# Cornell-RelaxML/QuIP

Measured on NVIDIA H100. Metric: tokens/sec 2-bit Llama-2-7B (per-layer eval path, seq 2048), higher is better.
Workload: dtype f16

## Files before the change

quip_b200/csrc/qgemm_tc.cu:

```cuda
#include <type_traits>

#include "tc_common.cuh"

namespace quip {

constexpr int TC_SMEM_MAX = 227 * 1024;

template <int BITS, int BN, bool DENSE, int RB = 1>
struct TcCfg {
  static constexpr int BM = TC_BM * RB;
  static constexpr int A_BYTES = DENSE ? TC_BM * TC_BK * 2 : (BM / SB_ROWS) * sb_words(BITS) * 4;
  static constexpr int B_BYTES = BN * TC_BK * 2;
  static constexpr int STAGE_BYTES = A_BYTES + B_BYTES;
  static constexpr int EPI_HALVES = BN * 72 > 64 * (BN + 8) ? BN * 72 : 64 * (BN + 8);
  static constexpr int EPI_BYTES = 2 * EPI_HALVES * 2;
  static constexpr int STAGES_FIT = (TC_SMEM_MAX - EPI_BYTES - 1024 - 256) / STAGE_BYTES;
  static constexpr int STAGES = STAGES_FIT < 16 ? STAGES_FIT : 16;
  static constexpr size_t SMEM = (size_t)STAGES * STAGE_BYTES + 1024  + 256  + EPI_BYTES;
  static_assert(STAGE_BYTES % 1024 == 0 && 2 * STAGES * 8 <= 256, "stage layout");
  static_assert(RB == 1 || (!DENSE && BN == 128), "256-row tiles: packed GEMM at BN = 128 only");
};

template <int BITS, int BN, bool DENSE, int RB = 1>
__global__ void __launch_bounds__(RB == 1 ? TC_THREADS : TC_THREADS_TALL, 1)
qgemm_tc_kernel(const __grid_constant__ CUtensorMap tmap_x, const __grid_constant__ CUtensorMap tmap_a,
                const float* __restrict__ scales, const float* __restrict__ zeros, const __half* __restrict__ bias,
                const float* __restrict__ xsum, __half* __restrict__ z, int M, int K, int N, int symmetric, int nblk,
                int shared_factor) {
  using C = TcCfg<BITS, BN, DENSE, RB>;
  extern __shared__ unsigned char smem_raw[];
  const uint32_t smem_base = (smem_u32(smem_raw) + 1023u) & ~1023u;
  unsigned char* smem_gen = smem_raw + (smem_base - smem_u32(smem_raw));
  uint64_t* bars = reinterpret_cast<uint64_t*>(smem_gen + (size_t)C::STAGES * C::STAGE_BYTES);
  uint64_t* full = bars;
  uint64_t* empty = bars + C::STAGES;
  __half* epi = reinterpret_cast<__half*>(smem_gen + (size_t)C::STAGES * C::STAGE_BYTES + 256);

  const int warp = threadIdx.x >> 5, lane = threadIdx.x & 31;
  const int tiles_n = DENSE ? (N + BN - 1) / BN : (N + C::BM - 1) / C::BM;
  const int tiles_m = DENSE ? (M + TC_BM - 1) / TC_BM : (M + BN - 1) / BN;
  const int per_blk = tiles_n * tiles_m;
  const int num_tiles = per_blk * nblk;
  const int KB = (K + TC_BK - 1) / TC_BK;
  const int64_t ldz = (int64_t)N * nblk;
  constexpr int TMA_WARP = TC_CONSUMER_WARPS;

  if (warp == TMA_WARP && lane == 0) {
    asm volatile("prefetch.tensormap [%0];" ::"l"(&tmap_x) : "memory");
    asm volatile("prefetch.tensormap [%0];" ::"l"(&tmap_a) : "memory");
    for (int s = 0; s < C::STAGES; ++s) {
      mbar_init(&full[s], 1);
      mbar_init(&empty[s], TC_CONSUMER_WARPS);
    }
    asm volatile("fence.mbarrier_init.release.cluster;" ::: "memory");
  }
  __syncthreads();

  if (RB == 1 ? warp == TMA_WARP : warp >= TMA_WARP) {
    if constexpr (RB == 2) asm volatile("setmaxnreg.dec.sync.aligned.u32 %0;" ::"n"(TC_TALL_PRODUCER_REGS));
    if (lane == 0 && (RB == 1 || warp == TMA_WARP)) {
      int s = 0;
      uint32_t ph = 0;
      for (int tile = blockIdx.x; tile < num_tiles; tile += gridDim.x) {
        const int blk = tile / per_blk, rr = tile % per_blk;
        const int m0 = (rr / tiles_n) * (DENSE ? TC_BM : BN), n0 = (rr % tiles_n) * (DENSE ? BN : C::BM);
        for (int kb = 0; kb < KB; ++kb) {
          mbar_wait(&empty[s], ph ^ 1u);
          unsigned char* stage = smem_gen + (size_t)s * C::STAGE_BYTES;
          if (DENSE) {
            mbar_arrive_expect_tx(&full[s], C::STAGE_BYTES);
            tma_load_2d(stage, &tmap_x, &full[s], blk * K + kb * TC_BK, m0);
            tma_load_3d(stage + C::A_BYTES, &tmap_a, &full[s], kb * TC_BK, n0, shared_factor ? 0 : blk);
          } else {
            const bool words = (kb & 1) == 0;
            mbar_arrive_expect_tx(&full[s], C::B_BYTES + (words ? C::A_BYTES : 0));
            if (words) tma_load_2d(stage, &tmap_a, &full[s], (kb >> 1) * sb_words(BITS), n0 / SB_ROWS);
            tma_load_2d(stage + C::A_BYTES, &tmap_x, &full[s], kb * TC_BK, m0);
          }
          if (++s == C::STAGES) { s = 0; ph ^= 1u; }
        }
      }
    }
  } else {
    if constexpr (RB == 2) asm volatile("setmaxnreg.inc.sync.aligned.u32 %0;" ::"n"(TC_TALL_CONSUMER_REGS));
    const int wg = warp >> 2, wtid = threadIdx.x & 127;
    const int frow = (warp & 3) * 16 + (lane >> 2);
    const int fcol = (lane & 3) * 2;
    __half* eb = epi + wg * C::EPI_HALVES;
    float acc[RB][BN / 2];
#pragma unroll
    for (int j = 0; j < BN / 2; ++j) acc[0][j] = 0.f;
    int s = 0;
    uint32_t ph = 0;
    auto advance = [&]() { if (++s == C::STAGES) { s = 0; ph ^= 1u; } };
    auto release = [&](int st) {
      __syncwarp();
      if (lane == 0) mbar_arrive(&empty[st]);
    };
    for (int tile = blockIdx.x; tile < num_tiles; tile += gridDim.x) {
      const int blk = tile / per_blk, rr = tile % per_blk;
      int prev = 0;
      const int n_base = (rr % tiles_n) * C::BM + wg * 64 * RB, m0 = (rr / tiles_n) * BN;
      float Pn[RB][2], Rn[RB][2], bn[RB][2];
      if constexpr (!DENSE) {
#pragma unroll
        for (int hf = 0; hf < RB; ++hf)
#pragma unroll
          for (int h = 0; h < 2; ++h) {
            const int n = n_base + 64 * hf + frow + 8 * h;
            Pn[hf][h] = 1.f; Rn[hf][h] = 0.f; bn[hf][h] = 0.f;
            if (n < N) {
              const float sc = scales[n];
              Pn[hf][h] = sc * (float)(1 << BITS);
              if (!symmetric) Rn[hf][h] = sc * (0.5f * (float)((1 << BITS) - 1)) - zeros[n];
              if (bias) bn[hf][h] = __half2float(bias[n]);
            }
          }
        if (!symmetric && wtid < BN / 32 && m0 + 32 * wtid < M)
          asm volatile("prefetch.global.L1 [%0];" ::"l"(xsum + m0 + 32 * wtid));
      }
      if constexpr (DENSE) {
        for (int kb = 0; kb < KB; ++kb) {
          mbar_wait(&full[s], ph);
          const uint32_t a_addr = smem_base + (uint32_t)(s * C::STAGE_BYTES);
          const uint64_t adesc = make_sw128_desc(a_addr + (uint32_t)(wg * 64 * 128));
          const uint64_t bdesc = make_sw128_desc(a_addr + C::A_BYTES);
          wgmma_fence();
#pragma unroll
          for (int k = 0; k < TC_BK / 16; ++k)
            wgmma_f16_ss<BN>(acc[0], adesc + (uint64_t)(2 * k), bdesc + (uint64_t)(2 * k), (kb | k) ? 1 : 0);
          wgmma_commit();
          wgmma_wait<1>();
          if (kb > 0) release(prev);
          prev = s;
          advance();
        }
      } else if constexpr (RB == 1) {
        const int g = lane >> 2, t = lane & 3;
        const uint32_t row_off = (uint32_t)(warp * sb_words(BITS) * 4);
        uint32_t w[row_words(BITS)];
        uint32_t fa[2][16];
        auto issue = [&](const uint32_t (&f)[16], int first) {
          const uint64_t bdesc = make_sw128_desc(smem_base + (uint32_t)(s * C::STAGE_BYTES) + C::A_BYTES);
          wgmma_fence();
#pragma unroll
          for (int k = 0; k < TC_BK / 16; ++k)
            wgmma_f16_rs<BN>(acc[0], &f[4 * k], bdesc + (uint64_t)(2 * k), (first && k == 0) ? 0 : 1);
          wgmma_commit();
        };
        auto load_words = [&]() {
          mbar_wait(&full[s], ph);
          tc_load_row_words<BITS>(smem_base + (uint32_t)(s * C::STAGE_BYTES) + row_off, g, w);
        };
        load_words();
        frag_natural<BITS, 0, 0>(w, t, &fa[0][0]);
        frag_natural<BITS, 0, 1>(w, t, &fa[0][4]);
        frag_natural<BITS, 1, 0>(w, t, &fa[0][8]);
        frag_natural<BITS, 1, 1>(w, t, &fa[0][12]);
        const int KSB = KB >> 1;
        for (int ksb = 0; ksb < KSB; ++ksb) {
          const int se = s;
          issue(fa[0], ksb == 0);
          wgmma_wait<1>();
          if (ksb > 0) release(prev);
          advance();
          mbar_wait(&full[s], ph);
          frag_natural<BITS, 2, 0>(w, t, &fa[1][0]);
          frag_natural<BITS, 2, 1>(w, t, &fa[1][4]);
          frag_natural<BITS, 3, 0>(w, t, &fa[1][8]);
          frag_natural<BITS, 3, 1>(w, t, &fa[1][12]);
          issue(fa[1], 0);
          wgmma_wait<1>();
          release(se);
          prev = s;
          advance();
          if (ksb + 1 < KSB) {
            load_words();
            frag_natural<BITS, 0, 0>(w, t, &fa[0][0]);
            frag_natural<BITS, 0, 1>(w, t, &fa[0][4]);
            frag_natural<BITS, 1, 0>(w, t, &fa[0][8]);
            frag_natural<BITS, 1, 1>(w, t, &fa[0][12]);
          }
        }
      } else {
        const int g = lane >> 2, t = lane & 3;
        const uint32_t row_off0 = (uint32_t)((wg * 8 + (warp & 3)) * sb_words(BITS) * 4);
        const uint32_t row_off1 = row_off0 + (uint32_t)(4 * sb_words(BITS) * 4);
        uint32_t w[row_words(BITS)];
        uint32_t fa[2][16];
        auto issue = [&](const uint32_t (&f)[16], float (&d)[BN / 2], int first) {
          const uint64_t bdesc = make_sw128_desc(smem_base + (uint32_t)(s * C::STAGE_BYTES) + C::A_BYTES);
          wgmma_fence();
#pragma unroll
          for (int k = 0; k < TC_BK / 16; ++k)
            wgmma_f16_rs<BN>(d, &f[4 * k], bdesc + (uint64_t)(2 * k), (first && k == 0) ? 0 : 1);
          wgmma_commit();
        };
        auto build = [&](auto odd, int se, uint32_t off, uint32_t (&f)[16]) {
          tc_load_row_words<BITS>(smem_base + (uint32_t)(se * C::STAGE_BYTES) + off, g, w);
          constexpr int c0 = decltype(odd)::value ? 2 : 0;
          frag_natural<BITS, c0, 0>(w, t, &f[0]);
          frag_natural<BITS, c0, 1>(w, t, &f[4]);
          frag_natural<BITS, c0 + 1, 0>(w, t, &f[8]);
          frag_natural<BITS, c0 + 1, 1>(w, t, &f[12]);
        };
        using Even = std::false_type;
        using Odd = std::true_type;
        mbar_wait(&full[s], ph);
        build(Even{}, s, row_off0, fa[0]);
        const int KSB = KB >> 1;
        for (int ksb = 0; ksb < KSB; ++ksb) {
          const int se = s;
          issue(fa[0], acc[0], ksb == 0);
          wgmma_wait<1>();
          if (ksb > 0) release(prev);
          build(Even{}, se, row_off1, fa[1]);
          issue(fa[1], acc[1], ksb == 0);
          wgmma_wait<1>();
          build(Odd{}, se, row_off0, fa[0]);
          advance();
          mbar_wait(&full[s], ph);
          issue(fa[0], acc[0], 0);
          wgmma_wait<1>();
          build(Odd{}, se, row_off1, fa[1]);
          release(se);
          issue(fa[1], acc[1], 0);
          wgmma_wait<1>();
          prev = s;
          advance();
          if (ksb + 1 < KSB) {
            mbar_wait(&full[s], ph);
            build(Even{}, s, row_off0, fa[0]);
          }
        }
      }
      wgmma_wait<0>();
      wgmma_fence_regs(acc[0]);
      if constexpr (RB == 2) wgmma_fence_regs(acc[RB - 1]);
      release(prev);

      if constexpr (DENSE) {
        constexpr int EP = BN + 8;
#pragma unroll
        for (int j = 0; j < BN / 2; j += 2) {
          const int r = frow + ((j & 2) ? 8 : 0), c = 8 * (j >> 2) + fcol;
          *reinterpret_cast<__half2*>(&eb[r * EP + c]) = __floats2half2_rn(acc[0][j], acc[0][j + 1]);
        }
        asm volatile("bar.sync %0, 128;" ::"r"(1 + wg) : "memory");
        const int m_base = (rr / tiles_n) * TC_BM + wg * 64, i0 = (rr % tiles_n) * BN;
        for (int idx = wtid; idx < 64 * (BN / 8); idx += 128) {
          const int r = idx / (BN / 8), v = idx % (BN / 8);
          const int m = m_base + r, i = i0 + 8 * v;
          if (m < M && i < N)
            *reinterpret_cast<uint4*>(z + (int64_t)m * ldz + (int64_t)blk * N + i) =
                *reinterpret_cast<const uint4*>(&eb[r * EP + 8 * v]);
        }
      } else {
        constexpr int EP = 72;
#pragma unroll
        for (int hf = 0; hf < RB; ++hf) {
#pragma unroll
          for (int j = 0; j < BN / 2; ++j) {
            const int h = (j >> 1) & 1, c = 8 * (j >> 2) + fcol + (j & 1), m = m0 + c;
            float v = Pn[hf][h] * acc[hf][j] + bn[hf][h];
            if (!symmetric) v += Rn[hf][h] * (m < M ? __ldg(&xsum[m]) : 0.f);
            eb[c * EP + frow + 8 * h] = __float2half_rn(v);
          }
          asm volatile("bar.sync %0, 128;" ::"r"(1 + wg) : "memory");
          for (int idx = wtid; idx < BN * 8; idx += 128) {
            const int c = idx >> 3, v = idx & 7;
            const int m = m0 + c, n = n_base + 64 * hf + 8 * v;
            if (m < M && n < N)
              *reinterpret_cast<uint4*>(z + (int64_t)m * ldz + n) = *reinterpret_cast<const uint4*>(&eb[c * EP + 8 * v]);
          }
          if (hf + 1 < RB) asm volatile("bar.sync %0, 128;" ::"r"(1 + wg) : "memory");
        }
      }
      asm volatile("bar.sync %0, 128;" ::"r"(1 + wg) : "memory");
    }
  }
}

typedef CUresult (*PFN_encodeTiled)(CUtensorMap*, CUtensorMapDataType, cuuint32_t, void*, const cuuint64_t*,
                                    const cuuint64_t*, const cuuint32_t*, const cuuint32_t*, CUtensorMapInterleave,
                                    CUtensorMapSwizzle, CUtensorMapL2promotion, CUtensorMapFloatOOBfill);

static PFN_encodeTiled get_encode() {
  static PFN_encodeTiled fn = nullptr;
  if (!fn) {
    void* p = nullptr;
    cudaDriverEntryPointQueryResult qres;
    if (cudaGetDriverEntryPoint("cuTensorMapEncodeTiled", &p, cudaEnableDefault, &qres) == cudaSuccess &&
        qres == cudaDriverEntryPointSuccess)
      fn = (PFN_encodeTiled)p;
  }
  return fn;
}

static int g_num_sms = 0;

int num_sms() {
  if (!g_num_sms) {
    int dev = 0;
    if (cudaGetDevice(&dev) != cudaSuccess ||
        cudaDeviceGetAttribute(&g_num_sms, cudaDevAttrMultiProcessorCount, dev) != cudaSuccess)
      g_num_sms = 132;
  }
  return g_num_sms;
}

int make_act_map(CUtensorMap* tmap, const void* x, int64_t rows, int64_t cols, int box_rows) {
  PFN_encodeTiled enc = get_encode();
  if (!enc) {
    set_error("cuTensorMapEncodeTiled is not available from the driver");
    return QUIP_ERR_CUDA;
  }
  cuuint64_t dims[2] = {(cuuint64_t)cols, (cuuint64_t)rows};
  cuuint64_t strides[1] = {(cuuint64_t)cols * sizeof(__half)};
  cuuint32_t box[2] = {(cuuint32_t)TC_BK, (cuuint32_t)box_rows};
  cuuint32_t estr[2] = {1, 1};
  CUresult r = enc(tmap, CU_TENSOR_MAP_DATA_TYPE_FLOAT16, 2, (void*)x, dims, strides, box, estr,
                   CU_TENSOR_MAP_INTERLEAVE_NONE, CU_TENSOR_MAP_SWIZZLE_128B, CU_TENSOR_MAP_L2_PROMOTION_L2_256B,
                   CU_TENSOR_MAP_FLOAT_OOB_FILL_NONE);
  if (r != CUDA_SUCCESS) {
    set_error("cuTensorMapEncodeTiled failed with CUresult %d (ptr=%p rows=%lld cols=%lld)", (int)r, x,
              (long long)rows, (long long)cols);
    return QUIP_ERR_CUDA;
  }
  return QUIP_OK;
}

static int make_words_map(CUtensorMap* tmap, const QuipLinearDesc* d, int rows) {
  PFN_encodeTiled enc = get_encode();
  if (!enc) {
    set_error("cuTensorMapEncodeTiled is not available from the driver");
    return QUIP_ERR_CUDA;
  }
  const int sbw = sb_words(d->bits);
  cuuint64_t dims[2] = {(cuuint64_t)(d->K / SB_K) * sbw, (cuuint64_t)(d->N / SB_ROWS)};
  cuuint64_t strides[1] = {dims[0] * sizeof(uint32_t)};
  cuuint32_t box[2] = {(cuuint32_t)sbw, (cuuint32_t)(rows / SB_ROWS)};
  cuuint32_t estr[2] = {1, 1};
  CUresult r = enc(tmap, CU_TENSOR_MAP_DATA_TYPE_UINT32, 2, (void*)d->qweight, dims, strides, box, estr,
                   CU_TENSOR_MAP_INTERLEAVE_NONE, CU_TENSOR_MAP_SWIZZLE_NONE, CU_TENSOR_MAP_L2_PROMOTION_L2_256B,
                   CU_TENSOR_MAP_FLOAT_OOB_FILL_NONE);
  if (r != CUDA_SUCCESS) {
    set_error("cuTensorMapEncodeTiled (packed words) failed with CUresult %d (N=%d K=%d bits=%d)", (int)r, d->N, d->K,
              d->bits);
    return QUIP_ERR_CUDA;
  }
  return QUIP_OK;
}

template <int BITS, int BN, int RB = 1>
static int launch_tc(const QuipLinearDesc* d, const __half* x, const float* xsum, const __half* bias, __half* z,
                     int M, cudaStream_t s) {
  using C = TcCfg<BITS, BN, false, RB>;
  CUtensorMap tmx, tmq;
  if (int e = make_act_map(&tmx, x, M, d->K, BN)) return e;
  if (int e = make_words_map(&tmq, d, C::BM)) return e;
  auto kern = qgemm_tc_kernel<BITS, BN, false, RB>;
  QUIP_CUDA(cudaFuncSetAttribute(kern, cudaFuncAttributeMaxDynamicSharedMemorySize, (int)C::SMEM));
  int tiles = ceil_div(d->N, C::BM) * ceil_div(M, BN);
  int grid = tiles < num_sms() ? tiles : num_sms();
  kern<<<grid, RB == 1 ? TC_THREADS : TC_THREADS_TALL, C::SMEM, s>>>(tmx, tmq, d->scales, d->zeros, bias, xsum, z, M, d->K, d->N,
                                         (d->flags & QUIP_FLAG_SYMMETRIC) ? 1 : 0, 1, 0);
  QUIP_LAUNCHED("qgemm_tc_kernel");
  return QUIP_OK;
}

template <int BN>
static int launch_tc_dense(const QuipPass* ps, const __half* in, __half* out, int M, int n, cudaStream_t s) {
  using C = TcCfg<2, BN, true>;
  PFN_encodeTiled enc = get_encode();
  CUtensorMap tmx, tma;
  if (int e = make_act_map(&tmx, in, M, n, TC_BM)) return e;
  const int p = ps->p;
  cuuint64_t dims[3] = {(cuuint64_t)p, (cuuint64_t)p, (cuuint64_t)(ps->shared ? 1 : ps->nblk)};
  cuuint64_t strides[2] = {(cuuint64_t)p * sizeof(__half), (cuuint64_t)p * p * sizeof(__half)};
  cuuint32_t box[3] = {(cuuint32_t)TC_BK, (cuuint32_t)BN, 1};
  cuuint32_t estr[3] = {1, 1, 1};
  CUresult r = enc(&tma, CU_TENSOR_MAP_DATA_TYPE_FLOAT16, 3, (void*)ps->factors, dims, strides, box, estr,
                   CU_TENSOR_MAP_INTERLEAVE_NONE, CU_TENSOR_MAP_SWIZZLE_128B, CU_TENSOR_MAP_L2_PROMOTION_L2_256B,
                   CU_TENSOR_MAP_FLOAT_OOB_FILL_NONE);
  if (r != CUDA_SUCCESS) {
    set_error("cuTensorMapEncodeTiled (factors) failed with CUresult %d (p=%d nblk=%d)", (int)r, p, ps->nblk);
    return QUIP_ERR_CUDA;
  }
  auto kern = qgemm_tc_kernel<2, BN, true>;
  QUIP_CUDA(cudaFuncSetAttribute(kern, cudaFuncAttributeMaxDynamicSharedMemorySize, (int)C::SMEM));
  int tiles = ceil_div(p, BN) * ceil_div(M, TC_BM) * ps->nblk;
  int grid = tiles < num_sms() ? tiles : num_sms();
  kern<<<grid, TC_THREADS, C::SMEM, s>>>(tmx, tma, nullptr, nullptr, nullptr, nullptr, out, M, p, p, 1,
                                         ps->nblk, ps->shared ? 1 : 0);
  QUIP_LAUNCHED("qgemm_tc_kernel<dense>");
  return QUIP_OK;
}

int pass_big_tc(const QuipPass* ps, const __half* in, __half* out, int64_t M, int n, cudaStream_t s) {
  QUIP_CHECK_ARG(!ps->strided && ps->p % 8 == 0 && n % 8 == 0, "tensor-core pass needs contiguous blocks, p %% 8 == 0");
  QUIP_CHECK_ARG((((uintptr_t)in | (uintptr_t)out | (uintptr_t)ps->factors) & 15) == 0, "tensor-core pass: unaligned pointer");
  return launch_tc_dense<128>(ps, in, out, (int)M, n, s);
}

int g_tc_rows = 0;

int qgemm_tc(const QuipLinearDesc* d, const __half* x, const float* xsum, const __half* bias, __half* z, int M,
             cudaStream_t s) {
  QUIP_CHECK_ARG((((uintptr_t)x | (uintptr_t)d->qweight) & 15) == 0,
                 "tensor-core path needs 16-byte aligned activations and packed words");
  const bool wide = M > 64;
  if (d->bits == 2 && wide) {
    const bool tall = g_tc_rows == 0 ? ceil_div(d->N, 2 * TC_BM) * ceil_div(M, 128) >= num_sms() : g_tc_rows == 256;
    return tall ? launch_tc<2, 128, 2>(d, x, xsum, bias, z, M, s) : launch_tc<2, 128>(d, x, xsum, bias, z, M, s);
  }
#define QUIP_TC(B)                                                            \
  if (d->bits == B)                                                           \
    return wide ? launch_tc<B, 128>(d, x, xsum, bias, z, M, s) : launch_tc<B, 64>(d, x, xsum, bias, z, M, s);
  QUIP_TC(2) QUIP_TC(3) QUIP_TC(4)
#undef QUIP_TC
  set_error("tensor-core kernel: unsupported bits=%d", d->bits);
  return QUIP_ERR_UNSUPPORTED;
}

}
```

quip_b200/csrc/tc_common.cuh:

```cuda
#pragma once
#include <cuda.h>

#include "common.cuh"

namespace quip {

constexpr int TC_BM = 128;
constexpr int TC_BK = 64;
constexpr int TC_CONSUMER_WARPS = 8;
constexpr int TC_THREADS = 32 * TC_CONSUMER_WARPS + 32;
constexpr int TC_THREADS_TALL = 32 * TC_CONSUMER_WARPS + 128;
constexpr int TC_TALL_PRODUCER_REGS = 40;
constexpr int TC_TALL_CONSUMER_REGS = 232;
constexpr uint32_t TC_WATCHDOG = 1u << 28;

__device__ __forceinline__ void mbar_init(uint64_t* bar, uint32_t count) {
  asm volatile("mbarrier.init.shared::cta.b64 [%0], %1;" ::"r"(smem_u32(bar)), "r"(count));
}
__device__ __forceinline__ void mbar_wait(uint64_t* bar, uint32_t parity) {
  uint32_t addr = smem_u32(bar), done = 0, spins = 0;
  while (true) {
    asm volatile(
        "{\n\t.reg .pred p;\n\t"
        "mbarrier.try_wait.parity.shared::cta.b64 p, [%1], %2;\n\t"
        "selp.u32 %0, 1, 0, p;\n\t}"
        : "=r"(done)
        : "r"(addr), "r"(parity)
        : "memory");
    if (done) break;
    if (++spins > TC_WATCHDOG) __trap();
  }
}
__device__ __forceinline__ void mbar_arrive(uint64_t* bar) {
  asm volatile("mbarrier.arrive.shared::cta.b64 _, [%0];" ::"r"(smem_u32(bar)) : "memory");
}
__device__ __forceinline__ void mbar_arrive_expect_tx(uint64_t* bar, uint32_t bytes) {
  asm volatile("mbarrier.arrive.expect_tx.shared::cta.b64 _, [%0], %1;" ::"r"(smem_u32(bar)), "r"(bytes) : "memory");
}
__device__ __forceinline__ void tma_load_2d(void* smem_dst, const CUtensorMap* map, uint64_t* bar, int c0, int c1) {
  asm volatile(
      "cp.async.bulk.tensor.2d.shared::cluster.global.mbarrier::complete_tx::bytes [%0], [%1, {%3, %4}], [%2];"
      ::"r"(smem_u32(smem_dst)), "l"(map), "r"(smem_u32(bar)), "r"(c0), "r"(c1)
      : "memory");
}
__device__ __forceinline__ void tma_load_3d(void* smem_dst, const CUtensorMap* map, uint64_t* bar, int c0, int c1, int c2) {
  asm volatile(
      "cp.async.bulk.tensor.3d.shared::cluster.global.mbarrier::complete_tx::bytes [%0], [%1, {%3, %4, %5}], [%2];"
      ::"r"(smem_u32(smem_dst)), "l"(map), "r"(smem_u32(bar)), "r"(c0), "r"(c1), "r"(c2)
      : "memory");
}

__device__ __forceinline__ uint64_t make_sw128_desc(uint32_t smem_addr) {
  uint64_t d = 0;
  d |= (uint64_t)((smem_addr & 0x3FFFFu) >> 4);
  d |= (uint64_t)1 << 16;
  d |= (uint64_t)(1024 >> 4) << 32;
  d |= (uint64_t)1 << 62;
  return d;
}

template <int N>
__device__ __forceinline__ void wgmma_f16_ss(float (&d)[N / 2], uint64_t adesc, uint64_t bdesc, int scale_d);
template <>
__device__ __forceinline__ void wgmma_f16_ss<64>(float (&d)[32], uint64_t adesc, uint64_t bdesc, int scale_d) {
  asm volatile(
      "{\n\t.reg .pred p;\n\t"
      "setp.ne.b32 p, %34, 0;\n\t"
      "wgmma.mma_async.sync.aligned.m64n64k16.f32.f16.f16 "
      "{%0,%1,%2,%3,%4,%5,%6,%7,%8,%9,%10,%11,%12,%13,%14,%15,%16,%17,%18,%19,%20,%21,%22,%23,%24,%25,%26,%27,%28,%29,%30,%31}, "
      "%32, %33, p, 1, 1, 0, 0;\n\t}"
      : "+f"(d[0]), "+f"(d[1]), "+f"(d[2]), "+f"(d[3]), "+f"(d[4]), "+f"(d[5]), "+f"(d[6]), "+f"(d[7]), "+f"(d[8]), "+f"(d[9]), "+f"(d[10]), "+f"(d[11]), "+f"(d[12]), "+f"(d[13]), "+f"(d[14]), "+f"(d[15]), "+f"(d[16]), "+f"(d[17]), "+f"(d[18]), "+f"(d[19]), "+f"(d[20]), "+f"(d[21]), "+f"(d[22]), "+f"(d[23]), "+f"(d[24]), "+f"(d[25]), "+f"(d[26]), "+f"(d[27]), "+f"(d[28]), "+f"(d[29]), "+f"(d[30]), "+f"(d[31])
      : "l"(adesc), "l"(bdesc), "r"(scale_d));
}

template <>
__device__ __forceinline__ void wgmma_f16_ss<128>(float (&d)[64], uint64_t adesc, uint64_t bdesc, int scale_d) {
  asm volatile(
      "{\n\t.reg .pred p;\n\t"
      "setp.ne.b32 p, %66, 0;\n\t"
      "wgmma.mma_async.sync.aligned.m64n128k16.f32.f16.f16 "
      "{%0,%1,%2,%3,%4,%5,%6,%7,%8,%9,%10,%11,%12,%13,%14,%15,%16,%17,%18,%19,%20,%21,%22,%23,%24,%25,%26,%27,%28,%29,%30,%31,%32,%33,%34,%35,%36,%37,%38,%39,%40,%41,%42,%43,%44,%45,%46,%47,%48,%49,%50,%51,%52,%53,%54,%55,%56,%57,%58,%59,%60,%61,%62,%63}, "
      "%64, %65, p, 1, 1, 0, 0;\n\t}"
      : "+f"(d[0]), "+f"(d[1]), "+f"(d[2]), "+f"(d[3]), "+f"(d[4]), "+f"(d[5]), "+f"(d[6]), "+f"(d[7]), "+f"(d[8]), "+f"(d[9]), "+f"(d[10]), "+f"(d[11]), "+f"(d[12]), "+f"(d[13]), "+f"(d[14]), "+f"(d[15]), "+f"(d[16]), "+f"(d[17]), "+f"(d[18]), "+f"(d[19]), "+f"(d[20]), "+f"(d[21]), "+f"(d[22]), "+f"(d[23]), "+f"(d[24]), "+f"(d[25]), "+f"(d[26]), "+f"(d[27]), "+f"(d[28]), "+f"(d[29]), "+f"(d[30]), "+f"(d[31]), "+f"(d[32]), "+f"(d[33]), "+f"(d[34]), "+f"(d[35]), "+f"(d[36]), "+f"(d[37]), "+f"(d[38]), "+f"(d[39]), "+f"(d[40]), "+f"(d[41]), "+f"(d[42]), "+f"(d[43]), "+f"(d[44]), "+f"(d[45]), "+f"(d[46]), "+f"(d[47]), "+f"(d[48]), "+f"(d[49]), "+f"(d[50]), "+f"(d[51]), "+f"(d[52]), "+f"(d[53]), "+f"(d[54]), "+f"(d[55]), "+f"(d[56]), "+f"(d[57]), "+f"(d[58]), "+f"(d[59]), "+f"(d[60]), "+f"(d[61]), "+f"(d[62]), "+f"(d[63])
      : "l"(adesc), "l"(bdesc), "r"(scale_d));
}
__device__ __forceinline__ void wgmma_fence() { asm volatile("wgmma.fence.sync.aligned;" ::: "memory"); }
__device__ __forceinline__ void wgmma_commit() { asm volatile("wgmma.commit_group.sync.aligned;" ::: "memory"); }
template <int PENDING>
__device__ __forceinline__ void wgmma_wait() { asm volatile("wgmma.wait_group.sync.aligned %0;" ::"n"(PENDING) : "memory"); }
template <int R>
__device__ __forceinline__ void wgmma_fence_regs(float (&d)[R]) {
#pragma unroll
  for (int i = 0; i < R; ++i) asm volatile("" : "+f"(d[i])::"memory");
}

template <int N>
__device__ __forceinline__ void wgmma_f16_rs(float (&d)[N / 2], const uint32_t* a, uint64_t bdesc, int scale_d);
template <>
__device__ __forceinline__ void wgmma_f16_rs<64>(float (&d)[32], const uint32_t* a, uint64_t bdesc, int scale_d) {
  asm volatile(
      "{\n\t.reg .pred p;\n\t"
      "setp.ne.b32 p, %37, 0;\n\t"
      "wgmma.mma_async.sync.aligned.m64n64k16.f32.f16.f16 "
      "{%0,%1,%2,%3,%4,%5,%6,%7,%8,%9,%10,%11,%12,%13,%14,%15,%16,%17,%18,%19,%20,%21,%22,%23,%24,%25,%26,%27,%28,%29,%30,%31}, "
      "{%32,%33,%34,%35}, %36, p, 1, 1, 0;\n\t}"
      : "+f"(d[0]), "+f"(d[1]), "+f"(d[2]), "+f"(d[3]), "+f"(d[4]), "+f"(d[5]), "+f"(d[6]), "+f"(d[7]), "+f"(d[8]), "+f"(d[9]), "+f"(d[10]), "+f"(d[11]), "+f"(d[12]), "+f"(d[13]), "+f"(d[14]), "+f"(d[15]), "+f"(d[16]), "+f"(d[17]), "+f"(d[18]), "+f"(d[19]), "+f"(d[20]), "+f"(d[21]), "+f"(d[22]), "+f"(d[23]), "+f"(d[24]), "+f"(d[25]), "+f"(d[26]), "+f"(d[27]), "+f"(d[28]), "+f"(d[29]), "+f"(d[30]), "+f"(d[31])
      : "r"(a[0]), "r"(a[1]), "r"(a[2]), "r"(a[3]), "l"(bdesc), "r"(scale_d));
}
template <>
__device__ __forceinline__ void wgmma_f16_rs<128>(float (&d)[64], const uint32_t* a, uint64_t bdesc, int scale_d) {
  asm volatile(
      "{\n\t.reg .pred p;\n\t"
      "setp.ne.b32 p, %69, 0;\n\t"
      "wgmma.mma_async.sync.aligned.m64n128k16.f32.f16.f16 "
      "{%0,%1,%2,%3,%4,%5,%6,%7,%8,%9,%10,%11,%12,%13,%14,%15,%16,%17,%18,%19,%20,%21,%22,%23,%24,%25,%26,%27,%28,%29,%30,%31,%32,%33,%34,%35,%36,%37,%38,%39,%40,%41,%42,%43,%44,%45,%46,%47,%48,%49,%50,%51,%52,%53,%54,%55,%56,%57,%58,%59,%60,%61,%62,%63}, "
      "{%64,%65,%66,%67}, %68, p, 1, 1, 0;\n\t}"
      : "+f"(d[0]), "+f"(d[1]), "+f"(d[2]), "+f"(d[3]), "+f"(d[4]), "+f"(d[5]), "+f"(d[6]), "+f"(d[7]), "+f"(d[8]), "+f"(d[9]), "+f"(d[10]), "+f"(d[11]), "+f"(d[12]), "+f"(d[13]), "+f"(d[14]), "+f"(d[15]), "+f"(d[16]), "+f"(d[17]), "+f"(d[18]), "+f"(d[19]), "+f"(d[20]), "+f"(d[21]), "+f"(d[22]), "+f"(d[23]), "+f"(d[24]), "+f"(d[25]), "+f"(d[26]), "+f"(d[27]), "+f"(d[28]), "+f"(d[29]), "+f"(d[30]), "+f"(d[31]), "+f"(d[32]), "+f"(d[33]), "+f"(d[34]), "+f"(d[35]), "+f"(d[36]), "+f"(d[37]), "+f"(d[38]), "+f"(d[39]), "+f"(d[40]), "+f"(d[41]), "+f"(d[42]), "+f"(d[43]), "+f"(d[44]), "+f"(d[45]), "+f"(d[46]), "+f"(d[47]), "+f"(d[48]), "+f"(d[49]), "+f"(d[50]), "+f"(d[51]), "+f"(d[52]), "+f"(d[53]), "+f"(d[54]), "+f"(d[55]), "+f"(d[56]), "+f"(d[57]), "+f"(d[58]), "+f"(d[59]), "+f"(d[60]), "+f"(d[61]), "+f"(d[62]), "+f"(d[63])
      : "r"(a[0]), "r"(a[1]), "r"(a[2]), "r"(a[3]), "l"(bdesc), "r"(scale_d));
}

template <int BITS>
__device__ __forceinline__ void tc_load_row_words(uint32_t rb, int g, uint32_t (&w)[row_words(BITS)]) {
  auto ld4 = [](uint32_t addr, uint32_t* d) {
    asm volatile("ld.shared.v4.b32 {%0,%1,%2,%3}, [%4];" : "=r"(d[0]), "=r"(d[1]), "=r"(d[2]), "=r"(d[3]) : "r"(addr));
  };
#pragma unroll
  for (int i = 0; i < 4; ++i) ld4(rb + (uint32_t)(16 * g + 4 * i) * 4u, &w[4 * i]);
  if constexpr (BITS == 3) {
#pragma unroll
    for (int i = 0; i < 2; ++i) ld4(rb + (uint32_t)(128 + 8 * g + 4 * i) * 4u, &w[16 + 4 * i]);
  } else if constexpr (BITS == 4) {
#pragma unroll
    for (int i = 0; i < 4; ++i) ld4(rb + (uint32_t)(128 + 16 * g + 4 * i) * 4u, &w[16 + 4 * i]);
  }
}
}
```

Before: 28330.

## Use stmatrix staging and TMA bulk stores for tall packed GEMM epilogue

```diff
diff --git a/quip_b200/csrc/qgemm_tc.cu b/quip_b200/csrc/qgemm_tc.cu
--- a/quip_b200/csrc/qgemm_tc.cu
+++ b/quip_b200/csrc/qgemm_tc.cu
@@ -13,28 +13,30 @@
   static constexpr int B_BYTES = BN * TC_BK * 2;
   static constexpr int STAGE_BYTES = A_BYTES + B_BYTES;
   static constexpr int EPI_HALVES = BN * 72 > 64 * (BN + 8) ? BN * 72 : 64 * (BN + 8);
-  static constexpr int EPI_BYTES = 2 * EPI_HALVES * 2;
+  static constexpr int STG_BOXES = RB == 2 ? 2 : 0;
+  static constexpr int BOX_BYTES = 64 * BN * 2;
+  static constexpr int EPI_BYTES = STG_BOXES ? 2 * STG_BOXES * BOX_BYTES : 2 * EPI_HALVES * 2;
   static constexpr int STAGES_FIT = (TC_SMEM_MAX - EPI_BYTES - 1024 - 256) / STAGE_BYTES;
   static constexpr int STAGES = STAGES_FIT < 16 ? STAGES_FIT : 16;
-  static constexpr size_t SMEM = (size_t)STAGES * STAGE_BYTES + 1024  + 256  + EPI_BYTES;
-  static_assert(STAGE_BYTES % 1024 == 0 && 2 * STAGES * 8 <= 256, "stage layout");
+  static constexpr size_t SMEM = (size_t)STAGES * STAGE_BYTES + 1024  + EPI_BYTES + 256 ;
+  static_assert(STAGE_BYTES % 1024 == 0 && EPI_BYTES % 1024 == 0 && 2 * STAGES * 8 <= 256, "stage layout");
   static_assert(RB == 1 || (!DENSE && BN == 128), "256-row tiles: packed GEMM at BN = 128 only");
 };
 
 template <int BITS, int BN, bool DENSE, int RB = 1>
 __global__ void __launch_bounds__(RB == 1 ? TC_THREADS : TC_THREADS_TALL, 1)
 qgemm_tc_kernel(const __grid_constant__ CUtensorMap tmap_x, const __grid_constant__ CUtensorMap tmap_a,
-                const float* __restrict__ scales, const float* __restrict__ zeros, const __half* __restrict__ bias,
+                const __grid_constant__ CUtensorMap tmap_z, const float* __restrict__ scales, const float* __restrict__ zeros, const __half* __restrict__ bias,
                 const float* __restrict__ xsum, __half* __restrict__ z, int M, int K, int N, int symmetric, int nblk,
                 int shared_factor) {
   using C = TcCfg<BITS, BN, DENSE, RB>;
   extern __shared__ unsigned char smem_raw[];
   const uint32_t smem_base = (smem_u32(smem_raw) + 1023u) & ~1023u;
   unsigned char* smem_gen = smem_raw + (smem_base - smem_u32(smem_raw));
-  uint64_t* bars = reinterpret_cast<uint64_t*>(smem_gen + (size_t)C::STAGES * C::STAGE_BYTES);
+  __half* epi = reinterpret_cast<__half*>(smem_gen + (size_t)C::STAGES * C::STAGE_BYTES);
+  uint64_t* bars = reinterpret_cast<uint64_t*>(smem_gen + (size_t)C::STAGES * C::STAGE_BYTES + C::EPI_BYTES);
   uint64_t* full = bars;
   uint64_t* empty = bars + C::STAGES;
-  __half* epi = reinterpret_cast<__half*>(smem_gen + (size_t)C::STAGES * C::STAGE_BYTES + 256);
 
   const int warp = threadIdx.x >> 5, lane = threadIdx.x & 31;
   const int tiles_n = DENSE ? (N + BN - 1) / BN : (N + C::BM - 1) / C::BM;
@@ -48,6 +50,7 @@
   if (warp == TMA_WARP && lane == 0) {
     asm volatile("prefetch.tensormap [%0];" ::"l"(&tmap_x) : "memory");
     asm volatile("prefetch.tensormap [%0];" ::"l"(&tmap_a) : "memory");
+    if (C::STG_BOXES) asm volatile("prefetch.tensormap [%0];" ::"l"(&tmap_z) : "memory");
     for (int s = 0; s < C::STAGES; ++s) {
       mbar_init(&full[s], 1);
       mbar_init(&empty[s], TC_CONSUMER_WARPS);
@@ -255,6 +258,49 @@
             *reinterpret_cast<uint4*>(z + (int64_t)m * ldz + (int64_t)blk * N + i) =
                 *reinterpret_cast<const uint4*>(&eb[r * EP + 8 * v]);
         }
+      } else if constexpr (C::STG_BOXES > 0) {
+        const uint32_t stg = smem_u32(epi) + (uint32_t)(wg * C::STG_BOXES * C::BOX_BYTES);
+        const int mi = lane >> 3, mk = lane & 7;
+        const uint32_t lane_off = (uint32_t)((8 * (mi >> 1) + mk) * 128 + (((2 * (warp & 3) + (mi & 1)) ^ mk) << 4));
+        if (wtid == 0) bulk_wait_all<true>();
+        asm volatile("bar.sync %0, 128;" ::"r"(1 + wg) : "memory");
+#pragma unroll
+        for (int qq = 0; qq < BN / 16; ++qq) {
+          float xs[2][2];
+#pragma unroll
+          for (int dq = 0; dq < 2; ++dq)
+#pragma unroll
+            for (int e = 0; e < 2; ++e) {
+              const int m = m0 + 8 * (2 * qq + dq) + fcol + e;
+              xs[dq][e] = symmetric ? 0.f : (m < M ? __ldg(&xsum[m]) : 0.f);
+            }
+#pragma unroll
+          for (int hf = 0; hf < RB; ++hf) {
+            uint32_t r[4];
+#pragma unroll
+            for (int ii = 0; ii < 4; ++ii) {
+              const int dq = ii >> 1, h = ii & 1, j = 4 * (2 * qq + dq) + 2 * h;
+              float v[2];
+#pragma unroll
+              for (int e = 0; e < 2; ++e) {
+                v[e] = Pn[hf][h] * acc[hf][j + e] + bn[hf][h];
+                if (!symmetric) v[e] += Rn[hf][h] * xs[dq][e];
+              }
+              r[ii] = pack_half2_rn(v[0], v[1]);
+            }
+            stmatrix_x4_trans(stg + (uint32_t)(hf * C::BOX_BYTES) + lane_off + (uint32_t)(qq * 16 * 128), r[0], r[1],
+                              r[2], r[3]);
+          }
+        }
+        fence_proxy_async_smem();
+        asm volatile("bar.sync %0, 128;" ::"r"(1 + wg) : "memory");
+        if (wtid == 0) {
+#pragma unroll
+          for (int hf = 0; hf < RB; ++hf)
+            if (n_base + 64 * hf < N) tma_store_2d(&tmap_z, stg + (uint32_t)(hf * C::BOX_BYTES), n_base + 64 * hf, m0);
+          bulk_commit();
+          if (tile + (int)gridDim.x >= num_tiles) bulk_wait_all<false>();
+        }
       } else {
         constexpr int EP = 72;
 #pragma unroll
@@ -276,7 +322,7 @@
           if (hf + 1 < RB) asm volatile("bar.sync %0, 128;" ::"r"(1 + wg) : "memory");
         }
       }
-      asm volatile("bar.sync %0, 128;" ::"r"(1 + wg) : "memory");
+      if constexpr (!C::STG_BOXES) asm volatile("bar.sync %0, 128;" ::"r"(1 + wg) : "memory");
     }
   }
 }
@@ -325,6 +371,26 @@
   if (r != CUDA_SUCCESS) {
     set_error("cuTensorMapEncodeTiled failed with CUresult %d (ptr=%p rows=%lld cols=%lld)", (int)r, x,
               (long long)rows, (long long)cols);
+    return QUIP_ERR_CUDA;
+  }
+  return QUIP_OK;
+}
+
+static int make_out_map(CUtensorMap* tmap, void* z, int64_t M, int64_t N, int box_tokens) {
+  PFN_encodeTiled enc = get_encode();
+  if (!enc) {
+    set_error("cuTensorMapEncodeTiled is not available from the driver");
+    return QUIP_ERR_CUDA;
+  }
+  cuuint64_t dims[2] = {(cuuint64_t)N, (cuuint64_t)M};
+  cuuint64_t strides[1] = {(cuuint64_t)N * sizeof(__half)};
+  cuuint32_t box[2] = {64, (cuuint32_t)box_tokens};
+  cuuint32_t estr[2] = {1, 1};
+  CUresult r = enc(tmap, CU_TENSOR_MAP_DATA_TYPE_FLOAT16, 2, z, dims, strides, box, estr, CU_TENSOR_MAP_INTERLEAVE_NONE,
+                   CU_TENSOR_MAP_SWIZZLE_128B, CU_TENSOR_MAP_L2_PROMOTION_NONE, CU_TENSOR_MAP_FLOAT_OOB_FILL_NONE);
+  if (r != CUDA_SUCCESS) {
+    set_error("cuTensorMapEncodeTiled (output) failed with CUresult %d (ptr=%p M=%lld N=%lld)", (int)r, z,
+              (long long)M, (long long)N);
     return QUIP_ERR_CUDA;
   }
   return QUIP_OK;
@@ -356,15 +422,17 @@
 static int launch_tc(const QuipLinearDesc* d, const __half* x, const float* xsum, const __half* bias, __half* z,
                      int M, cudaStream_t s) {
   using C = TcCfg<BITS, BN, false, RB>;
-  CUtensorMap tmx, tmq;
+  CUtensorMap tmx, tmq, tmz = {};
   if (int e = make_act_map(&tmx, x, M, d->K, BN)) return e;
   if (int e = make_words_map(&tmq, d, C::BM)) return e;
+  if (C::STG_BOXES)
+    if (int e = make_out_map(&tmz, z, M, d->N, BN)) return e;
   auto kern = qgemm_tc_kernel<BITS, BN, false, RB>;
   QUIP_CUDA(cudaFuncSetAttribute(kern, cudaFuncAttributeMaxDynamicSharedMemorySize, (int)C::SMEM));
   int tiles = ceil_div(d->N, C::BM) * ceil_div(M, BN);
   int grid = tiles < num_sms() ? tiles : num_sms();
-  kern<<<grid, RB == 1 ? TC_THREADS : TC_THREADS_TALL, C::SMEM, s>>>(tmx, tmq, d->scales, d->zeros, bias, xsum, z, M, d->K, d->N,
-                                         (d->flags & QUIP_FLAG_SYMMETRIC) ? 1 : 0, 1, 0);
+  kern<<<grid, RB == 1 ? TC_THREADS : TC_THREADS_TALL, C::SMEM, s>>>(tmx, tmq, tmz, d->scales, d->zeros, bias, xsum, z, M,
+                                                                      d->K, d->N, (d->flags & QUIP_FLAG_SYMMETRIC) ? 1 : 0, 1, 0);
   QUIP_LAUNCHED("qgemm_tc_kernel");
   return QUIP_OK;
 }
@@ -373,7 +441,7 @@
 static int launch_tc_dense(const QuipPass* ps, const __half* in, __half* out, int M, int n, cudaStream_t s) {
   using C = TcCfg<2, BN, true>;
   PFN_encodeTiled enc = get_encode();
-  CUtensorMap tmx, tma;
+  CUtensorMap tmx, tma, unused = {};
   if (int e = make_act_map(&tmx, in, M, n, TC_BM)) return e;
   const int p = ps->p;
   cuuint64_t dims[3] = {(cuuint64_t)p, (cuuint64_t)p, (cuuint64_t)(ps->shared ? 1 : ps->nblk)};
@@ -391,7 +459,7 @@
   QUIP_CUDA(cudaFuncSetAttribute(kern, cudaFuncAttributeMaxDynamicSharedMemorySize, (int)C::SMEM));
   int tiles = ceil_div(p, BN) * ceil_div(M, TC_BM) * ps->nblk;
   int grid = tiles < num_sms() ? tiles : num_sms();
-  kern<<<grid, TC_THREADS, C::SMEM, s>>>(tmx, tma, nullptr, nullptr, nullptr, nullptr, out, M, p, p, 1,
+  kern<<<grid, TC_THREADS, C::SMEM, s>>>(tmx, tma, unused, nullptr, nullptr, nullptr, nullptr, out, M, p, p, 1,
                                          ps->nblk, ps->shared ? 1 : 0);
   QUIP_LAUNCHED("qgemm_tc_kernel<dense>");
   return QUIP_OK;
@@ -407,8 +475,8 @@
 
 int qgemm_tc(const QuipLinearDesc* d, const __half* x, const float* xsum, const __half* bias, __half* z, int M,
              cudaStream_t s) {
-  QUIP_CHECK_ARG((((uintptr_t)x | (uintptr_t)d->qweight) & 15) == 0,
-                 "tensor-core path needs 16-byte aligned activations and packed words");
+  QUIP_CHECK_ARG((((uintptr_t)x | (uintptr_t)d->qweight | (uintptr_t)z) & 15) == 0,
+                 "tensor-core path needs 16-byte aligned activations, packed words and output");
   const bool wide = M > 64;
   if (d->bits == 2 && wide) {
     const bool tall = g_tc_rows == 0 ? ceil_div(d->N, 2 * TC_BM) * ceil_div(M, 128) >= num_sms() : g_tc_rows == 256;
diff --git a/quip_b200/csrc/tc_common.cuh b/quip_b200/csrc/tc_common.cuh
--- a/quip_b200/csrc/tc_common.cuh
+++ b/quip_b200/csrc/tc_common.cuh
@@ -48,6 +48,27 @@
       "cp.async.bulk.tensor.3d.shared::cluster.global.mbarrier::complete_tx::bytes [%0], [%1, {%3, %4, %5}], [%2];"
       ::"r"(smem_u32(smem_dst)), "l"(map), "r"(smem_u32(bar)), "r"(c0), "r"(c1), "r"(c2)
       : "memory");
+}
+
+__device__ __forceinline__ void tma_store_2d(const CUtensorMap* map, uint32_t smem_src, int c0, int c1) {
+  asm volatile("cp.async.bulk.tensor.2d.global.shared::cta.bulk_group [%0, {%2, %3}], [%1];"
+               ::"l"(map), "r"(smem_src), "r"(c0), "r"(c1) : "memory");
+}
+__device__ __forceinline__ void bulk_commit() { asm volatile("cp.async.bulk.commit_group;" ::: "memory"); }
+template <bool READ>
+__device__ __forceinline__ void bulk_wait_all() {
+  if constexpr (READ) asm volatile("cp.async.bulk.wait_group.read 0;" ::: "memory");
+  else asm volatile("cp.async.bulk.wait_group 0;" ::: "memory");
+}
+__device__ __forceinline__ void fence_proxy_async_smem() { asm volatile("fence.proxy.async.shared::cta;" ::: "memory"); }
+__device__ __forceinline__ uint32_t pack_half2_rn(float lo, float hi) {
+  uint32_t r;
+  asm("cvt.rn.f16x2.f32 %0, %1, %2;" : "=r"(r) : "f"(hi), "f"(lo));
+  return r;
+}
+__device__ __forceinline__ void stmatrix_x4_trans(uint32_t addr, uint32_t r0, uint32_t r1, uint32_t r2, uint32_t r3) {
+  asm volatile("stmatrix.sync.aligned.m8n8.x4.trans.shared.b16 [%0], {%1, %2, %3, %4};"
+               ::"r"(addr), "r"(r0), "r"(r1), "r"(r2), "r"(r3) : "memory");
 }
 
 __device__ __forceinline__ uint64_t make_sw128_desc(uint32_t smem_addr) {
```

Result: faster. 28670, median of 6 (+1.2%).
